# paipaoso/pytorch-operator-1

Hardware: AMD Instinct MI355X
Metric: samples/sec MNIST DDP (higher is better)
Workload: dtype fp32; 1 GPU; model=mnist-cnn (reference examples/mnist/mnist.py Net, 431,080 params), global_batch=64, per_rank_batch=64, optimizer=SGD lr=0.01 momentum=0.5, parallelism=dp1, impl=fused, sampler=none (every rank its own batch stream, reference-equivalent), backend=none

## Files before the change

pytorch_operator_1_amd/csrc/kernels/mnist_kernels.hip:

```cpp
#include <stdlib.h>

#include "mfma_f32.h"
#include "sgd_f32.h"
#include "xgmi_ar.h"

#ifndef PTO_STAMP
#define PTO_STAMP(k) ((void)0)
#define PTO_STAMP_SCOPE()
#endif

namespace {

constexpr int C1 = 20, C2 = 50, P1 = 12, F1OUT = 500, F1IN = 800, NCLS = 10;
constexpr int A1P = C1 * P1 * P1;

PTO_DEV void relu_pool4(const float v[4], float& out, uint8_t& code) {
  float m = v[0];
  int a = 0;
#pragma unroll
  for (int r = 1; r < 4; ++r)
    if (v[r] > m) { m = v[r]; a = r; }
  if (m > 0.f) { out = m; code = (uint8_t)a; }
  else { out = 0.f; code = 4; }
}

PTO_DEV const float* batch_ptr(const float* base, const long long* bidx, int per_batch) {
  return bidx ? base + (size_t)(*bidx) * per_batch : base;
}

struct LazyConv1 {
  const float* g;
  const float* m;
  const int* pending;
  SgdArgs a;
  int bias_off;
  float* xout;
  float* w2out;
  const float* rep;
  int nrep, rep_stride;
};
constexpr int C1_MAXREP = 256;
constexpr int REP_CHUNK = 16;
struct Conv1Commit {
  float* p;
  float* g;
  float* m;
  int n;
  const int* pending;
  SgdArgs a;
  float* rep;
  int nrep, rep_stride;
  int* zero_word;
};

PTO_DEV void commit4(const Conv1Commit& cm, int i, float lr) {
  if (cm.nrep <= 1) {
    sgd_flat4(cm.p, cm.g, cm.m, i, lr, cm.a);
    return;
  }
  float4 pv = *reinterpret_cast<float4*>(cm.p + i);
  float4 mv = *reinterpret_cast<float4*>(cm.m + i);
  float4 gs = *reinterpret_cast<const float4*>(cm.g + i);
  for (int r0 = 0; r0 < cm.nrep - 1; r0 += REP_CHUNK) {
    float4 v[REP_CHUNK];
#pragma unroll
    for (int r = 0; r < REP_CHUNK; ++r)
      v[r] = *reinterpret_cast<const float4*>(cm.rep + (size_t)min(r0 + r, cm.nrep - 2) * cm.rep_stride + i);
#pragma unroll
    for (int r = 0; r < REP_CHUNK; ++r) {
      if (r0 + r >= cm.nrep - 1) break;
      gs.x += v[r].x; gs.y += v[r].y; gs.z += v[r].z; gs.w += v[r].w;
      *reinterpret_cast<float4*>(cm.rep + (size_t)(r0 + r) * cm.rep_stride + i) = float4{0.f, 0.f, 0.f, 0.f};
    }
  }
  sgd_elem(pv.x, gs.x, mv.x, lr, cm.a.mom, cm.a.wd, cm.a.gscale, cm.a.nesterov);
  sgd_elem(pv.y, gs.y, mv.y, lr, cm.a.mom, cm.a.wd, cm.a.gscale, cm.a.nesterov);
  sgd_elem(pv.z, gs.z, mv.z, lr, cm.a.mom, cm.a.wd, cm.a.gscale, cm.a.nesterov);
  sgd_elem(pv.w, gs.w, mv.w, lr, cm.a.mom, cm.a.wd, cm.a.gscale, cm.a.nesterov);
  *reinterpret_cast<float4*>(cm.p + i) = pv;
  *reinterpret_cast<float4*>(cm.m + i) = mv;
  *reinterpret_cast<float4*>(cm.g + i) = float4{0.f, 0.f, 0.f, 0.f};
}

PTO_DEV float rep_sum(const float* __restrict__ rep, int nrep, int stride, int i, bool live, float s0) {
  float s = s0;
  for (int r0 = 0; r0 < nrep - 1; r0 += REP_CHUNK) {
    float v[REP_CHUNK];
#pragma unroll
    for (int r = 0; r < REP_CHUNK; ++r) v[r] = rep[(size_t)min(r0 + r, nrep - 2) * stride + i];
#pragma unroll
    for (int r = 0; r < REP_CHUNK; ++r) s += (live && r0 + r < nrep - 1) ? v[r] : 0.f;
  }
  return s;
}

__global__ __launch_bounds__(256) void k_conv1_fwd(const float* __restrict__ x, const float* __restrict__ w,
                                                   const float* __restrict__ bias, float* __restrict__ out,
                                                   uint8_t* __restrict__ code, int B,
                                                   const long long* __restrict__ bidx) {
  __shared__ float ws[C1 * 25];
  __shared__ float bs[C1];
  const int idx = blockIdx.x * 256 + threadIdx.x;
  const bool active = idx < B * 720;
  const int b = idx / 720, rem = idx - b * 720, cg = rem / 144, pix = rem - cg * 144;
  const int ph = pix / 12, pw = pix - ph * 12;
  float p[6][6];
  x = batch_ptr(x, bidx, B * 784);
  const float* xb = x + (active ? b * 784 + (2 * ph) * 28 + 2 * pw : 0);
#pragma unroll
  for (int r = 0; r < 6; ++r)
#pragma unroll
    for (int c = 0; c < 6; ++c) p[r][c] = xb[r * 28 + c];
  for (int i = threadIdx.x; i < C1 * 25; i += 256) ws[i] = w[i];
  if (threadIdx.x < C1) bs[threadIdx.x] = bias[threadIdx.x];
  __syncthreads();
  if (!active) return;
#pragma unroll
  for (int cc = 0; cc < 4; ++cc) {
    const int oc = cg * 4 + cc;
    const float* wc = ws + oc * 25;
    float v[4];
#pragma unroll
    for (int q = 0; q < 4; ++q) {
      const int dy = q >> 1, dx = q & 1;
      float s = bs[oc];
#pragma unroll
      for (int kh = 0; kh < 5; ++kh)
#pragma unroll
        for (int kw = 0; kw < 5; ++kw) s = fmaf(p[dy + kh][dx + kw], wc[kh * 5 + kw], s);
      v[q] = s;
    }
    float o;
    uint8_t cd;
    relu_pool4(v, o, cd);
    const int oi = ((b * C1 + oc) * P1 + ph) * P1 + pw;
    out[oi] = o;
    code[oi] = cd;
  }
}

constexpr int WS_LD = 502;
__global__ __launch_bounds__(256) void k_conv2_fwd(const float* __restrict__ a1p, const float* __restrict__ w2,
                                                   const float* __restrict__ b2, float* __restrict__ a2p,
                                                   uint8_t* __restrict__ code2, int B) {
  __shared__ float ws[16 * WS_LD];
  __shared__ __attribute__((aligned(16))) float in_s[A1P];
  const int b = blockIdx.x >> 2, nt = blockIdx.x & 3;
  const int tid = threadIdx.x;
  {
    const int nrows = min(16, C2 - nt * 16);
    const float4* wsrc = reinterpret_cast<const float4*>(w2 + nt * 16 * 500);
    const float4* isrc = reinterpret_cast<const float4*>(a1p + b * A1P);
    float4 wv[8], iv[3];
#pragma unroll
    for (int q = 0; q < 8; ++q) {
      const int e = tid + 256 * q;
      wv[q] = (e < nrows * 125) ? wsrc[e] : float4{0.f, 0.f, 0.f, 0.f};
    }
#pragma unroll
    for (int q = 0; q < 3; ++q) {
      const int e = tid + 256 * q;
      iv[q] = (e < A1P / 4) ? isrc[e] : float4{0.f, 0.f, 0.f, 0.f};
    }
#pragma unroll
    for (int q = 0; q < 8; ++q) {
      const int e = tid + 256 * q;
      if (e < 2000) {
        const int row = e / 125, col = (e - row * 125) * 4;
        float* d = ws + row * WS_LD + col;
        d[0] = wv[q].x; d[1] = wv[q].y; d[2] = wv[q].z; d[3] = wv[q].w;
      }
    }
#pragma unroll
    for (int q = 0; q < 3; ++q) {
      const int e = tid + 256 * q;
      if (e < A1P / 4) reinterpret_cast<float4*>(in_s)[e] = iv[q];
    }
  }
  __syncthreads();
  const int t = tid >> 6, lane = tid & 63;
  const int i = lane & 15, g = lane >> 4;
  const int pw = i >> 2, dy = (i >> 1) & 1, dx = i & 1;
  const int n = nt * 16 + (lane & 15);
  const float* wl = ws + (lane & 15) * WS_LD + 5 * g;
  const float* il = in_s + (2 * t + dy) * 12 + 2 * pw + dx;
  f32x4 acc0 = zero4(), acc1 = zero4();
#pragma unroll
  for (int G = 0; G < 25; ++G) {
    const int R = 4 * G + g;
    const int ic = R / 5, kh = R - ic * 5;
    const float* arow = il + ic * 144 + kh * 12;
    const float* brow = wl + 20 * G;
    acc0 = mfma16x16x4(arow[0], brow[0], acc0);
    acc1 = mfma16x16x4(arow[1], brow[1], acc1);
    acc0 = mfma16x16x4(arow[2], brow[2], acc0);
    acc1 = mfma16x16x4(arow[3], brow[3], acc1);
    acc0 = mfma16x16x4(arow[4], brow[4], acc0);
  }
  const f32x4 acc = acc0 + acc1;
  if (n >= C2 || b >= B) return;
  const float bn = b2[n];
  float v[4] = {acc[0] + bn, acc[1] + bn, acc[2] + bn, acc[3] + bn};
  float o;
  uint8_t cd;
  relu_pool4(v, o, cd);
  const int oi = b * F1IN + n * 16 + t * 4 + (lane >> 4);
  a2p[oi] = o;
  code2[oi] = cd;
}

struct ArRole {
  const pto_ar::ArPeers* peers;
  long long off, n4;
  int rank, world, chan, nblk;
  uint32_t* epochs;
  int* err;
  long long timeout;
  pto_ar::ArSgd f;
  int* ready;
};

template <bool SYS>
struct ParamView {
  const float* p;
  __amdgpu_buffer_rsrc_t r;
  PTO_DEV ParamView(const float* base, int n) : p(base) {
    if constexpr (SYS) r = __builtin_amdgcn_make_buffer_rsrc(const_cast<float*>(base), 0, n * 4, 0x00020000);
  }
  PTO_DEV float operator[](int i) const {
    if constexpr (SYS)
      return __builtin_bit_cast(float, __builtin_amdgcn_raw_buffer_load_b32(r, i * 4, 0, pto_ar::AUX_SYS));
    else
      return p[i];
  }
  PTO_DEV float4 v4(int i4) const {
    if constexpr (SYS)
      return __builtin_bit_cast(float4, __builtin_amdgcn_raw_buffer_load_b128(r, i4 * 16, 0, pto_ar::AUX_SYS));
    else
      return reinterpret_cast<const float4*>(p)[i4];
  }
};

PTO_DEV void wait_conv_role(const ArRole& cv) {
  const long long t0 = wall_clock64();
  for (;;) {
    const int r = __hip_atomic_load(cv.ready, __ATOMIC_RELAXED, __HIP_MEMORY_SCOPE_AGENT);
    const int ev = __hip_atomic_load(cv.err, __ATOMIC_RELAXED, __HIP_MEMORY_SCOPE_AGENT);
    if (r >= cv.nblk || ev != 0) break;
    if (wall_clock64() - t0 > cv.timeout) {
      atomicOr(cv.err, 16);
      break;
    }
    __builtin_amdgcn_s_sleep(1);
  }
}
constexpr int W1PLD = 52;
template <int NTH, int ARM = 0>
__global__ __launch_bounds__(NTH, ARM ? 2 * NTH / 256 : 1) void k_conv12_fwd2_t(
    const float* __restrict__ x, const float* __restrict__ w1, const float* __restrict__ b1,
    const float* __restrict__ w2, const float* __restrict__ b2, float* __restrict__ a1p, uint8_t* __restrict__ code1,
    float* __restrict__ a2p, uint8_t* __restrict__ code2, int B, const long long* __restrict__ bidx, LazyConv1 lz,
    ArRole ar, ArRole cv) {
  int bx = (int)blockIdx.x;
  if constexpr (ARM != 0) {
    if (bx < cv.nblk + ar.nblk) {
      PTO_STAMP_SCOPE();
      __shared__ float4 ar_lds[NTH];
      if (bx < cv.nblk)
        pto_ar::ar_role_oneshot_sgd<ARM == 2, NTH>(cv.peers, cv.off, cv.n4, cv.rank, cv.world, cv.chan, cv.epochs,
                                                   cv.err, cv.timeout, cv.f, bx, ar_lds, cv.ready);
      else
        pto_ar::ar_role_sgd<ARM == 2, NTH>(ar.peers, ar.off, ar.n4, ar.rank, ar.world, ar.chan, ar.epochs, ar.err,
                                           ar.timeout, ar.f, bx - cv.nblk, ar_lds);
      return;
    }
    bx -= cv.nblk + ar.nblk;
  }
  constexpr bool SYS = ARM != 0;
  __shared__ float ws[16 * WS_LD];
  __shared__ __attribute__((aligned(16))) float in_s[A1P];
  __shared__ __attribute__((aligned(16))) float xs[784];
  __shared__ float b1s[C1];
  __shared__ __attribute__((aligned(16))) float w1p[(C1 / 2) * W1PLD];
  constexpr int NWV = NTH / 64, NPART = NTH / 256;
  __shared__ __attribute__((aligned(16))) float red[(NPART - 1) * 1024];
  PTO_STAMP_SCOPE();
  const int b = bx >> 2, nt = bx & 3;
  const int tid = threadIdx.x;
  {
    x = batch_ptr(x, bidx, B * 784);
    const float4 xv = tid < 196 ? reinterpret_cast<const float4*>(x + b * 784)[tid] : float4{0.f, 0.f, 0.f, 0.f};
    if constexpr (ARM != 0) {
      if (tid == 0) wait_conv_role(cv);
      __syncthreads();
      PTO_STAMP(5);
    }
    const int nrows = min(16, C2 - nt * 16);
    const ParamView<SYS> wsrc(w2 + nt * 16 * 500, nrows * 500);
    float4 wv[2048 / NTH];
#pragma unroll
    for (int q = 0; q < 2048 / NTH; ++q) {
      const int e = tid + NTH * q;
      wv[q] = (e < nrows * 125) ? wsrc.v4(e) : float4{0.f, 0.f, 0.f, 0.f};
    }
    constexpr int QW1 = (C1 * 26 + NTH - 1) / NTH;
    float wq[QW1], gq[QW1], mq[QW1];
    const ParamView<SYS> w1v(w1, C1 * 25), b1v(b1, C1);
#pragma unroll
    for (int q = 0; q < QW1; ++q) {
      const int e = tid + NTH * q;
      wq[q] = e < C1 * 25 ? w1v[e] : (e < C1 * 26 ? b1v[e - C1 * 25] : 0.f);
    }
    int pend = 0;
    float lr = 0.f;
    if (lz.pending) {
      pend = *lz.pending;
      lr = *lz.a.lr;
#pragma unroll
      for (int q = 0; q < QW1; ++q) {
        const int e = tid + NTH * q;
        const int fi = e < C1 * 25 ? e : lz.bias_off + (e - C1 * 25);
        const float gsum = rep_sum(lz.rep, lz.nrep, lz.rep_stride, e < C1 * 26 ? fi : 0, e < C1 * 26,
                                   e < C1 * 26 ? lz.g[fi] : 0.f);
        gq[q] = gsum;
        mq[q] = e < C1 * 26 ? lz.m[fi] : 0.f;
      }
    }
    if (pend) {
#pragma unroll
      for (int q = 0; q < QW1; ++q) sgd_elem(wq[q], gq[q], mq[q], lr, lz.a.mom, lz.a.wd, lz.a.gscale, lz.a.nesterov);
    }
#pragma unroll
    for (int q = 0; q < 2048 / NTH; ++q) {
      const int e = tid + NTH * q;
      if (e < 2000) {
        const int row = e / 125, col = (e - row * 125) * 4;
        float* d = ws + row * WS_LD + col;
        d[0] = wv[q].x; d[1] = wv[q].y; d[2] = wv[q].z; d[3] = wv[q].w;
      }
    }
    if (tid < 196) {
      reinterpret_cast<float4*>(xs)[tid] = xv;
      if (lz.xout && nt == 0) reinterpret_cast<float4*>(lz.xout + b * 784)[tid] = xv;
    }
    if (lz.w2out && b == 0) {
#pragma unroll
      for (int q = 0; q < 2048 / NTH; ++q) {
        const int e = tid + NTH * q;
        if (e < nrows * 125) reinterpret_cast<float4*>(lz.w2out + nt * 16 * 500)[e] = wv[q];
      }
    }
#pragma unroll
    for (int q = 0; q < QW1; ++q) {
      const int e = tid + NTH * q;
      if (e < C1 * 25) {
        const int oc = e / 25, k = e - oc * 25;
        w1p[(oc >> 1) * W1PLD + 2 * k + (oc & 1)] = wq[q];
      } else if (e < C1 * 26) {
        b1s[e - C1 * 25] = wq[q];
      }
    }
  }
  __syncthreads();
  PTO_STAMP(1);
  const int wid = tid >> 6, lane = tid & 63;
  static_assert(NTH == 1024, "F12 is laid out for 16 waves");
  constexpr int CPT = 2;
  constexpr int NPAIR = C1 / CPT, NFULL = 2 * NPAIR, NTASK = NFULL + (NPAIR + 3) / 4;
  for (int si = 0; si < 2; ++si) {
    const int task = wid + NWV * si;
    if (task >= NTASK) break;
    int cg, pix;
    bool live = true;
    if (task < NFULL) {
      cg = task >> 1;
      pix = (task & 1) * 64 + lane;
    } else {
      cg = (task - NFULL) * 4 + (lane >> 4);
      pix = 128 + (lane & 15);
      live = cg < NPAIR;
      cg = min(cg, NPAIR - 1);
    }
    static_assert(CPT == 2, "w1p interleaves channel pairs");
    float wp[W1PLD], bz[CPT];
#pragma unroll
    for (int j = 0; j < W1PLD / 4; ++j) {
      const float4 v = *reinterpret_cast<const float4*>(w1p + cg * W1PLD + 4 * j);
      wp[4 * j] = v.x; wp[4 * j + 1] = v.y; wp[4 * j + 2] = v.z; wp[4 * j + 3] = v.w;
    }
#pragma unroll
    for (int cc = 0; cc < CPT; ++cc) bz[cc] = b1s[cg * CPT + cc];
    if (!live) continue;
    const int ph = pix / 12, pw = pix - ph * 12;
    float p[6][6];
#pragma unroll
    for (int r = 0; r < 6; ++r)
#pragma unroll
      for (int c = 0; c < 6; c += 2) {
        const float2 v = *reinterpret_cast<const float2*>(xs + (2 * ph + r) * 28 + 2 * pw + c);
        p[r][c] = v.x;
        p[r][c + 1] = v.y;
      }
    static_assert(CPT == 2, "conv1 full tasks pack two channels");
    f32x2 s2[4];
#pragma unroll
    for (int q = 0; q < 4; ++q) {
      const int dy = q >> 1, dx = q & 1;
      f32x2 acc2 = f32x2{bz[0], bz[1]};
#pragma unroll
      for (int kh = 0; kh < 5; ++kh)
#pragma unroll
        for (int kw = 0; kw < 5; ++kw) {
          const float pv = p[dy + kh][dx + kw];
          acc2 = __builtin_elementwise_fma(f32x2{pv, pv}, f32x2{wp[2 * (kh * 5 + kw)], wp[2 * (kh * 5 + kw) + 1]},
                                           acc2);
        }
      s2[q] = acc2;
    }
#pragma unroll
    for (int cc = 0; cc < CPT; ++cc) {
      const int oc = cg * CPT + cc;
      float v[4];
#pragma unroll
      for (int q = 0; q < 4; ++q) v[q] = s2[q][cc];
      float o;
      uint8_t cd;
      relu_pool4(v, o, cd);
      in_s[oc * 144 + pix] = o;
      if (nt == 0) {
        a1p[b * A1P + oc * 144 + pix] = o;
        code1[b * A1P + oc * 144 + pix] = cd;
      }
    }
  }
  __syncthreads();
  PTO_STAMP(2);
  const int t = wid & 3, half = wid >> 2;
  const int i = lane & 15, g = lane >> 4;
  const int pw = i >> 2, dy = (i >> 1) & 1, dx = i & 1;
  const int n = nt * 16 + (lane & 15);
  const float* wl = ws + (lane & 15) * WS_LD + 5 * g;
  const float* il = in_s + (2 * t + dy) * 12 + 2 * pw + dx;
  f32x4 acc0 = zero4(), acc1 = zero4();
  auto group = [&](int G) {
    const int R = 4 * G + g;
    const int ic = R / 5, kh = R - ic * 5;
    const float* arow = il + ic * 144 + kh * 12;
    const float* brow = wl + 20 * G;
    acc0 = mfma16x16x4(arow[0], brow[0], acc0);
    acc1 = mfma16x16x4(arow[1], brow[1], acc1);
    acc0 = mfma16x16x4(arow[2], brow[2], acc0);
    acc1 = mfma16x16x4(arow[3], brow[3], acc1);
    acc0 = mfma16x16x4(arow[4], brow[4], acc0);
  };
  if (NPART == 2) {
    if (half == 0) {
#pragma unroll
      for (int G = 0; G < 13; ++G) group(G);
    } else {
#pragma unroll
      for (int G = 13; G < 25; ++G) group(G);
    }
  } else {
    if (half == 0) {
#pragma unroll
      for (int G = 0; G < 7; ++G) group(G);
    } else {
      const int g0 = 7 + 6 * (half - 1);
#pragma unroll
      for (int G = 0; G < 6; ++G) group(g0 + G);
    }
  }
  f32x4 acc = acc0 + acc1;
  if (half != 0) {
#pragma unroll
    for (int rr = 0; rr < 4; ++rr) red[(half - 1) * 1024 + t * 256 + rr * 64 + lane] = acc[rr];
  }
  __syncthreads();
  PTO_STAMP(3);
  if (half != 0) return;
#pragma unroll
  for (int pp = 0; pp < NPART - 1; ++pp)
#pragma unroll
    for (int rr = 0; rr < 4; ++rr) acc[rr] += red[pp * 1024 + t * 256 + rr * 64 + lane];
  if (n >= C2 || b >= B) return;
  const float bn = ParamView<SYS>(b2, C2)[n];
  float v[4] = {acc[0] + bn, acc[1] + bn, acc[2] + bn, acc[3] + bn};
  float o;
  uint8_t cd;
  relu_pool4(v, o, cd);
  const int oi = b * F1IN + n * 16 + t * 4 + (lane >> 4);
  a2p[oi] = o;
  code2[oi] = cd;
}

struct EpiBiasRelu {
  const float* bias; float* out; int ld; bool relu;
  PTO_DEV void operator()(int m, int n, float v) const {
    v += bias ? bias[n] : 0.f;
    out[m * ld + n] = relu ? fmaxf(v, 0.f) : v;
  }
};
struct EpiStore {
  float* out; int ld;
  PTO_DEV void operator()(int m, int n, float v) const { out[m * ld + n] = v; }
};


__global__ __launch_bounds__(256) void k_linear_fwd(const float* __restrict__ x, const float* __restrict__ w,
                                                    const float* __restrict__ bias, float* __restrict__ y, int M,
                                                    int N, int K, int relu) {
  __shared__ float red[4 * 256];
  block_gemm_splitk4<LAY_ROWK, LAY_ROWK>(x, K, w, K, M, N, K, blockIdx.x, red,
                                          EpiBiasRelu{bias, y, N, relu != 0});
}

constexpr int RED_RR = 80, RED_W = 4 * RED_RR;
PTO_DEV int red_slot(int t) { return ((t >> 4) & 3) * RED_RR + (t >> 6) * 16 + (t & 15); }

PTO_DEV int xcd_tile(int i, int T, bool on) { return (on && !(T & 7)) ? (i & 7) * (T >> 3) + (i >> 3) : i; }

__global__ __launch_bounds__(1024) void k_linear_fwd_vec16(const float* __restrict__ x, const float* __restrict__ w,
                                                           const float* __restrict__ bias, float* __restrict__ y,
                                                           int M, int N, int K, int relu) {
  __shared__ float red[16 * RED_W];
  PTO_STAMP_SCOPE();
  const int mtiles = (M + 15) >> 4;
  const int tile = xcd_tile(blockIdx.x, gridDim.x, true);
  const int mt = tile % mtiles, nt = tile / mtiles;
  const int wv = threadIdx.x >> 6, lane = threadIdx.x & 63;
  const int kc = (((K + 15) / 16) + 15) & ~15;
  const f32x4 acc = wave_tile_16x16<LAY_ROWK, LAY_ROWK, 4, true, true>(x, K, w, K, M, N, K, mt * 16, nt * 16,
                                                                       wv * kc, (wv + 1) * kc);
#pragma unroll
  for (int rr = 0; rr < 4; ++rr) red[wv * RED_W + rr * RED_RR + lane] = acc[rr];
  PTO_STAMP(1);
  __syncthreads();
  PTO_STAMP(2);
  const int t = threadIdx.x;
  if (t < 256) {
    float v = 0.f;
#pragma unroll
    for (int q = 0; q < 16; ++q) v += red[q * RED_W + red_slot(t)];
    const int m = mt * 16 + (t >> 4), n = nt * 16 + (t & 15);
    if (m < M && n < N) EpiBiasRelu{bias, y, N, relu != 0}(m, n, v);
  }
}

template <int NW>
__global__ __launch_bounds__(NW * 64) void k_fc1_fwd_split2(const float* __restrict__ x, const float* __restrict__ w,
                                                          float* __restrict__ h, int M) {
  constexpr int KW = ((F1IN / 2 + NW - 1) / NW + 15) / 16 * 16;
  __shared__ float red[NW * RED_W];
  PTO_STAMP_SCOPE();
  const int mtiles = (M + 15) >> 4;
  const int i = blockIdx.x, xcd = i & 7, j = i >> 3;
  const int nt = 4 * xcd + j / (2 * mtiles), mt = (j >> 1) % mtiles, half = j & 1;
  const int wv = threadIdx.x >> 6, lane = threadIdx.x & 63;
  constexpr int KH = F1IN / 2;
  const int kb = half * KH + wv * KW, ke = min(kb + KW, (half + 1) * KH);
  const f32x4 acc = wave_tile_16x16<LAY_ROWK, LAY_ROWK, KW / 16, true, true>(x, F1IN, w, F1IN, M, F1OUT, F1IN,
                                                                             mt * 16, nt * 16, kb, ke);
#pragma unroll
  for (int rr = 0; rr < 4; ++rr) red[wv * RED_W + rr * RED_RR + lane] = acc[rr];
  PTO_STAMP(1);
  __syncthreads();
  PTO_STAMP(2);
  const int t = threadIdx.x;
  if (t < 256) {
    float v = 0.f;
#pragma unroll
    for (int q = 0; q < NW; ++q) v += red[q * RED_W + red_slot(t)];
    const int m = mt * 16 + (t >> 4), n = nt * 16 + (t & 15);
    if (m < M && n < F1OUT) atomicAdd(h + m * F1OUT + n, v);
  }
}

__global__ __launch_bounds__(256) void k_linear_bwd_data(const float* __restrict__ dy, const float* __restrict__ w,
                                                         float* __restrict__ dx, int M, int N, int K) {
  __shared__ float red[4 * 256];
  block_gemm_splitk4<LAY_ROWK, LAY_KROW>(dy, N, w, K, M, K, N, blockIdx.x, red, EpiStore{dx, K});
}

__global__ __launch_bounds__(256) void k_linear_bwd_weight(const float* __restrict__ dy, const float* __restrict__ x,
                                                           float* __restrict__ dw, int M, int N, int K) {
  block_gemm_4tiles<LAY_KROW, LAY_KROW>(dy, N, x, K, N, K, M, blockIdx.x, EpiStore{dw, K});
}

__global__ __launch_bounds__(256) void k_colsum(const float* __restrict__ dy, float* __restrict__ db, int M, int N) {
  __shared__ float red[256];
  block_colsum64(dy, N, M, N, blockIdx.x * 64, red, db);
}

__global__ __launch_bounds__(256) void k_relu_bwd(const float* __restrict__ g, const float* __restrict__ y,
                                                  float* __restrict__ out, int n) {
  const int i = blockIdx.x * 256 + threadIdx.x;
  if (i < n) out[i] = y[i] > 0.f ? g[i] : 0.f;
}

PTO_DEV void fc2_ce_row(int row, int lane, const float* __restrict__ h1, const float* __restrict__ w,
                        const float* __restrict__ bias, const int64_t* __restrict__ labels,
                        float* __restrict__ logp, float* __restrict__ loss_rows, float* __restrict__ dlogits,
                        float* __restrict__ dh1, int B, float inv_b, const long long* __restrict__ bidx) {
  float h[8], wv[NCLS][8], bz[NCLS];
#pragma unroll
  for (int j = 0; j < 8; ++j) {
    const int k = lane + 64 * j;
    h[j] = k < F1OUT ? h1[row * F1OUT + k] : 0.f;
#pragma unroll
    for (int c = 0; c < NCLS; ++c) wv[c][j] = k < F1OUT ? w[c * F1OUT + k] : 0.f;
  }
#pragma unroll
  for (int c = 0; c < NCLS; ++c) bz[c] = bias[c];
  int y = 0;
  if (labels) {
    if (bidx) labels += (size_t)(*bidx) * B;
    y = (int)labels[row];
  }
  float z[NCLS];
#pragma unroll
  for (int c = 0; c < NCLS; ++c) {
    float s = 0.f;
#pragma unroll
    for (int j = 0; j < 8; ++j) s = fmaf(h[j], wv[c][j], s);
    z[c] = s;
  }
  {
    float h8[8], h4[4], h2[2], h1;
#pragma unroll
    for (int k = 0; k < 8; ++k) {
      const bool up = lane & 32;
      const float a0 = z[k], a1 = k + 8 < NCLS ? z[k + 8] : 0.f;
      h8[k] = (up ? a1 : a0) + __shfl_xor(up ? a0 : a1, 32, 64);
    }
#pragma unroll
    for (int k = 0; k < 4; ++k) {
      const bool up = lane & 16;
      h4[k] = (up ? h8[k + 4] : h8[k]) + __shfl_xor(up ? h8[k] : h8[k + 4], 16, 64);
    }
#pragma unroll
    for (int k = 0; k < 2; ++k) {
      const bool up = lane & 8;
      h2[k] = (up ? h4[k + 2] : h4[k]) + __shfl_xor(up ? h4[k] : h4[k + 2], 8, 64);
    }
    {
      const bool up = lane & 4;
      h1 = (up ? h2[1] : h2[0]) + __shfl_xor(up ? h2[0] : h2[1], 4, 64);
    }
    h1 += __shfl_xor(h1, 2, 64);
    h1 += __shfl_xor(h1, 1, 64);
#pragma unroll
    for (int c = 0; c < NCLS; ++c) {
      const int src = ((c >> 3) & 1) * 32 + ((c >> 2) & 1) * 16 + ((c >> 1) & 1) * 8 + (c & 1) * 4;
      z[c] = __int_as_float(__builtin_amdgcn_readlane(__float_as_int(h1), src));
    }
  }
#pragma unroll
  for (int c = 0; c < NCLS; ++c) z[c] += bz[c];
  float mx = z[0];
#pragma unroll
  for (int c = 1; c < NCLS; ++c) mx = fmaxf(mx, z[c]);
  float se = 0.f;
#pragma unroll
  for (int c = 0; c < NCLS; ++c) se += __expf(z[c] - mx);
  const float lse = mx + __logf(se);
  float dl[NCLS];
#pragma unroll
  for (int c = 0; c < NCLS; ++c) dl[c] = (__expf(z[c] - lse) - (c == y ? 1.f : 0.f)) * inv_b;
  if (lane < NCLS) {
    float zl = z[0], dd = dl[0];
#pragma unroll
    for (int c = 1; c < NCLS; ++c)
      if (lane == c) { zl = z[c]; dd = dl[c]; }
    if (logp) logp[row * NCLS + lane] = zl - lse;
    if (dlogits) dlogits[row * NCLS + lane] = dd;
  }
  if (lane == 0 && loss_rows) {
    float zy = z[0];
#pragma unroll
    for (int c = 1; c < NCLS; ++c)
      if (c == y) zy = z[c];
    loss_rows[row] = lse - zy;
  }
  if (!dh1) return;
#pragma unroll
  for (int j = 0; j < 8; ++j) {
    const int k = lane + 64 * j;
    if (k < F1OUT) {
      float s = 0.f;
#pragma unroll
      for (int c = 0; c < NCLS; ++c) s = fmaf(dl[c], wv[c][j], s);
      dh1[row * F1OUT + k] = h[j] > 0.f ? s : 0.f;
    }
  }
}

__global__ __launch_bounds__(256) void k_fc2_ce(const float* __restrict__ h1, const float* __restrict__ w,
                                                const float* __restrict__ bias, const int64_t* __restrict__ labels,
                                                float* __restrict__ logp, float* __restrict__ loss_rows,
                                                float* __restrict__ dlogits, float* __restrict__ dh1, int B,
                                                float inv_b, const long long* __restrict__ bidx) {
  const int row = blockIdx.x * 4 + (threadIdx.x >> 6), lane = threadIdx.x & 63;
  if (row >= B) return;
  fc2_ce_row(row, lane, h1, w, bias, labels, logp, loss_rows, dlogits, dh1, B, inv_b, bidx);
}

constexpr int FDX_WAVES = 16;
constexpr int DLS_LD = 20;

struct BatchStage {
  const float* x;
  float* xnext;
  long long nb;
  int n4;
};
constexpr int STAGE_BLOCKS = 4;

__global__ __launch_bounds__(FDX_WAVES * 64) void k_fc2_ce_dx_mf(
    const float* __restrict__ h1, const float* __restrict__ w2, const float* __restrict__ b2,
    const int64_t* __restrict__ labels, const float* __restrict__ w1, float* __restrict__ loss_rows,
    float* __restrict__ dlogits, float* __restrict__ dh1, float* __restrict__ da2p, int B, float inv_b,
    const long long* __restrict__ bidx, Conv1Commit cm, BatchStage st, const float* __restrict__ b1,
    float* __restrict__ h1out) {
  constexpr int HLD = F1OUT;
  __shared__ __attribute__((aligned(16))) float hs[16 * HLD];
  __shared__ __attribute__((aligned(16))) float w2s[NCLS * HLD];
  __shared__ float red[FDX_WAVES * RED_W];
  __shared__ __attribute__((aligned(16))) float dls[16 * DLS_LD];
  const int mtiles = (B + 15) >> 4, ntiles = (F1IN + 15) >> 4;
  const int t = threadIdx.x;
  PTO_STAMP_SCOPE();
  if (blockIdx.x > (unsigned)(mtiles * ntiles)) {
    const long long nb = (*bidx + 1) % st.nb;
    const float4* src = reinterpret_cast<const float4*>(st.x) + nb * st.n4;
    float4* dst = reinterpret_cast<float4*>(st.xnext);
    const int j0 = (blockIdx.x - mtiles * ntiles - 1) * (FDX_WAVES * 64) + t;
    constexpr int STRIDE = STAGE_BLOCKS * FDX_WAVES * 64;
    for (int i0 = j0; i0 < st.n4; i0 += 4 * STRIDE) {
      const int i1 = i0 + STRIDE, i2 = i0 + 2 * STRIDE, i3 = i0 + 3 * STRIDE;
      const float4 v0 = src[i0];
      const float4 v1 = src[i1 < st.n4 ? i1 : i0];
      const float4 v2 = src[i2 < st.n4 ? i2 : i0];
      const float4 v3 = src[i3 < st.n4 ? i3 : i0];
      dst[i0] = v0;
      if (i1 < st.n4) dst[i1] = v1;
      if (i2 < st.n4) dst[i2] = v2;
      if (i3 < st.n4) dst[i3] = v3;
    }
    return;
  }
  if (blockIdx.x == (unsigned)(mtiles * ntiles)) {
    if (cm.zero_word && t == 0) *cm.zero_word = 0;
    if (cm.pending) {
      const int pend = *cm.pending;
      const float lr = *cm.a.lr;
      if (pend)
        for (int i = 4 * t; i < cm.n; i += 4 * FDX_WAVES * 64) commit4(cm, i, lr);
    }
    return;
  }
  const int tile = xcd_tile(blockIdx.x, mtiles * ntiles, true);
  const int mt = tile % mtiles, nt = tile / mtiles;
  const int w = t >> 6, lane = t & 63;
  const int r = lane & 15, gq = lane >> 4;
  constexpr int KC = ((F1OUT + FDX_WAVES - 1) / FDX_WAVES + 15) & ~15;
  constexpr int NGK = KC / 16;
  constexpr int H4 = 16 * F1OUT / 4, W4 = NCLS * F1OUT / 4;
  constexpr int NT = FDX_WAVES * 64;
  static_assert(F1OUT % 4 == 0 && H4 <= 2 * NT && W4 <= 2 * NT, "staging assumes two float4 rounds");
  const int kb = w * KC, kend = min((w + 1) * KC, F1OUT);
  const int nrow = min(16, B - mt * 16);
  const float4* hg = reinterpret_cast<const float4*>(h1 + (size_t)mt * 16 * F1OUT);
  const float4* wg = reinterpret_cast<const float4*>(w2);
  const float4 z4 = make_float4(0.f, 0.f, 0.f, 0.f);
  const int h4n = nrow * (F1OUT / 4);
  float4 hv0 = t < h4n ? hg[t] : float4(z4);
  float4 hv1 = (t + NT < H4 && t + NT < h4n) ? hg[t + NT] : float4(z4);
  float4 bb0 = z4, bb1 = z4;
  if (b1) {
    const float4* b4 = reinterpret_cast<const float4*>(b1);
    constexpr int RB = F1OUT / 4;
    bb0 = b4[t % RB];
    bb1 = b4[(t + NT) % RB];
  }
  const float4 wv0 = t < W4 ? wg[t] : float4(z4);
  const float4 wv1 = t + NT < W4 ? wg[t + NT] : float4(z4);
  float bw[NGK][4];
// ... 1401 lines not shown
```

Measured before the change: 1.922 million samples/s.

## Split conv2 blocks by output-row half instead of channel quarter to cut redundant conv1

In the non-allreduce path, each of the four blocks per sample now covers 32 output channels and half of the conv2 output rows, instead of 16 channels over all rows. Each block then only needs the conv1 pixels for its half (an overlapping 112 of 144), so conv1 runs in one round of tasks instead of two, which cuts conv1 work that was duplicated across the four blocks. In exchange each block holds and loads twice as much w2 into shared memory, which adds shared-memory footprint and global weight traffic.

```diff
diff --git a/pytorch_operator_1_amd/csrc/kernels/mnist_kernels.hip b/pytorch_operator_1_amd/csrc/kernels/mnist_kernels.hip
--- a/pytorch_operator_1_amd/csrc/kernels/mnist_kernels.hip
+++ b/pytorch_operator_1_amd/csrc/kernels/mnist_kernels.hip
@@ -277,7 +277,9 @@
     bx -= cv.nblk + ar.nblk;
   }
   constexpr bool SYS = ARM != 0;
-  __shared__ float ws[16 * WS_LD];
+  constexpr bool SPLIT = ARM == 0;
+  constexpr int NTILE = SPLIT ? 2 : 1;
+  __shared__ float ws[NTILE * 16 * WS_LD];
   __shared__ __attribute__((aligned(16))) float in_s[A1P];
   __shared__ __attribute__((aligned(16))) float xs[784];
   __shared__ float b1s[C1];
@@ -285,8 +287,13 @@
   constexpr int NWV = NTH / 64, NPART = NTH / 256;
   __shared__ __attribute__((aligned(16))) float red[(NPART - 1) * 1024];
   PTO_STAMP_SCOPE();
-  const int b = bx >> 2, nt = bx & 3;
+  const int b = bx >> 2;
+  const int hp = SPLIT ? (bx >> 1) & 1 : 0;
+  const int ch0 = SPLIT ? (bx & 1) * 32 : (bx & 3) * 16;
+  const bool own_a1 = SPLIT ? (bx & 1) == 0 : (bx & 3) == 0;
+  const bool own_x = (bx & 3) == 0, own_w2 = b == 0 && hp == 0;
   const int tid = threadIdx.x;
+  const int nrows = min(16 * NTILE, C2 - ch0);
   {
     x = batch_ptr(x, bidx, B * 784);
     const float4 xv = tid < 196 ? reinterpret_cast<const float4*>(x + b * 784)[tid] : float4{0.f, 0.f, 0.f, 0.f};
@@ -295,11 +302,11 @@
       __syncthreads();
       PTO_STAMP(5);
     }
-    const int nrows = min(16, C2 - nt * 16);
-    const ParamView<SYS> wsrc(w2 + nt * 16 * 500, nrows * 500);
-    float4 wv[2048 / NTH];
-#pragma unroll
-    for (int q = 0; q < 2048 / NTH; ++q) {
+    const ParamView<SYS> wsrc(w2 + ch0 * 500, nrows * 500);
+    constexpr int QW2 = NTILE * 2048 / NTH;
+    float4 wv[QW2];
+#pragma unroll
+    for (int q = 0; q < QW2; ++q) {
       const int e = tid + NTH * q;
       wv[q] = (e < nrows * 125) ? wsrc.v4(e) : float4{0.f, 0.f, 0.f, 0.f};
     }
@@ -331,9 +338,9 @@
       for (int q = 0; q < QW1; ++q) sgd_elem(wq[q], gq[q], mq[q], lr, lz.a.mom, lz.a.wd, lz.a.gscale, lz.a.nesterov);
     }
 #pragma unroll
-    for (int q = 0; q < 2048 / NTH; ++q) {
+    for (int q = 0; q < QW2; ++q) {
       const int e = tid + NTH * q;
-      if (e < 2000) {
+      if (e < NTILE * 2000) {
         const int row = e / 125, col = (e - row * 125) * 4;
         float* d = ws + row * WS_LD + col;
         d[0] = wv[q].x; d[1] = wv[q].y; d[2] = wv[q].z; d[3] = wv[q].w;
@@ -341,13 +348,13 @@
     }
     if (tid < 196) {
       reinterpret_cast<float4*>(xs)[tid] = xv;
-      if (lz.xout && nt == 0) reinterpret_cast<float4*>(lz.xout + b * 784)[tid] = xv;
-    }
-    if (lz.w2out && b == 0) {
-#pragma unroll
-      for (int q = 0; q < 2048 / NTH; ++q) {
+      if (lz.xout && own_x) reinterpret_cast<float4*>(lz.xout + b * 784)[tid] = xv;
+    }
+    if (lz.w2out && own_w2) {
+#pragma unroll
+      for (int q = 0; q < QW2; ++q) {
         const int e = tid + NTH * q;
-        if (e < nrows * 125) reinterpret_cast<float4*>(lz.w2out + nt * 16 * 500)[e] = wv[q];
+        if (e < nrows * 125) reinterpret_cast<float4*>(lz.w2out + ch0 * 500)[e] = wv[q];
       }
     }
 #pragma unroll
@@ -366,13 +373,24 @@
   const int wid = tid >> 6, lane = tid & 63;
   static_assert(NTH == 1024, "F12 is laid out for 16 waves");
   constexpr int CPT = 2;
-  constexpr int NPAIR = C1 / CPT, NFULL = 2 * NPAIR, NTASK = NFULL + (NPAIR + 3) / 4;
-  for (int si = 0; si < 2; ++si) {
+  constexpr int NPAIR = C1 / CPT, NFULL = SPLIT ? NPAIR : 2 * NPAIR;
+  constexpr int NTASK = NFULL + (SPLIT ? NPAIR / 2 : (NPAIR + 3) / 4);
+  static_assert(!SPLIT || (NPAIR % 2 == 0 && NTASK <= NWV), "split conv1: whole tail tasks, one round");
+  for (int si = 0; si < (NTASK + NWV - 1) / NWV; ++si) {
     const int task = wid + NWV * si;
     if (task >= NTASK) break;
     int cg, pix;
-    bool live = true;
-    if (task < NFULL) {
+    bool live = true, keep = own_a1;
+    if constexpr (SPLIT) {
+      if (task < NFULL) {
+        cg = task;
+        pix = 48 * hp + lane;
+      } else {
+        cg = (task - NFULL) * 2 + (lane >> 5);
+        pix = 48 * hp + 64 + (lane & 31);
+      }
+      keep = own_a1 && (hp == 0 ? pix < 72 : pix >= 72);
+    } else if (task < NFULL) {
       cg = task >> 1;
       pix = (task & 1) * 64 + lane;
     } else {
@@ -427,7 +445,7 @@
       uint8_t cd;
       relu_pool4(v, o, cd);
       in_s[oc * 144 + pix] = o;
-      if (nt == 0) {
+      if (keep) {
         a1p[b * A1P + oc * 144 + pix] = o;
         code1[b * A1P + oc * 144 + pix] = cd;
       }
@@ -435,11 +453,12 @@
   }
   __syncthreads();
   PTO_STAMP(2);
-  const int t = wid & 3, half = wid >> 2;
+  const int slot = wid & 3, half = wid >> 2;
+  const int t = SPLIT ? 2 * hp + (wid & 1) : slot, tile = SPLIT ? (wid >> 1) & 1 : 0;
   const int i = lane & 15, g = lane >> 4;
   const int pw = i >> 2, dy = (i >> 1) & 1, dx = i & 1;
-  const int n = nt * 16 + (lane & 15);
-  const float* wl = ws + (lane & 15) * WS_LD + 5 * g;
+  const int n = ch0 + tile * 16 + (lane & 15);
+  const float* wl = ws + (tile * 16 + (lane & 15)) * WS_LD + 5 * g;
   const float* il = in_s + (2 * t + dy) * 12 + 2 * pw + dx;
   f32x4 acc0 = zero4(), acc1 = zero4();
   auto group = [&](int G) {
@@ -474,7 +493,7 @@
   f32x4 acc = acc0 + acc1;
   if (half != 0) {
 #pragma unroll
-    for (int rr = 0; rr < 4; ++rr) red[(half - 1) * 1024 + t * 256 + rr * 64 + lane] = acc[rr];
+    for (int rr = 0; rr < 4; ++rr) red[(half - 1) * 1024 + slot * 256 + rr * 64 + lane] = acc[rr];
   }
   __syncthreads();
   PTO_STAMP(3);
@@ -482,7 +501,7 @@
 #pragma unroll
   for (int pp = 0; pp < NPART - 1; ++pp)
 #pragma unroll
-    for (int rr = 0; rr < 4; ++rr) acc[rr] += red[pp * 1024 + t * 256 + rr * 64 + lane];
+    for (int rr = 0; rr < 4; ++rr) acc[rr] += red[pp * 1024 + slot * 256 + rr * 64 + lane];
   if (n >= C2 || b >= B) return;
   const float bn = ParamView<SYS>(b2, C2)[n];
   float v[4] = {acc[0] + bn, acc[1] + bn, acc[2] + bn, acc[3] + bn};
```

Measured after the change: 1.921 million samples/s. No clear change (-0.1%).
